# BurntSushi/suffix

Hardware: AMD Instinct MI355X
Metric: MB of input text/sec for SuffixTable::new (SA-IS+LCP), 1 GPU; bit-exact SA (higher is better)
Workload: dtype u32; 1 GPU; 100000000 B synthetic DNA (sigma=4, uniform, splitmix64) per GPU, u32 indices, device-resident text -> device SA; text_bytes_total=100000000

## Files before the change

### suffix_amd/csrc/sfx_radix.hip

```cpp
#include <stdio.h>
#include <type_traits>
#include <stdlib.h>

#include "sfx_host.hpp"

namespace sfx {

constexpr uint32_t kStatusAgg = 1u << 30;
constexpr uint32_t kStatusPrefix = 2u << 30;
constexpr uint32_t kStatusValue = (1u << 30) - 1u;
constexpr int kMaxPasses = 8;
constexpr unsigned kHistAllGrid = 1024;

struct SrcE64 {
    static constexpr bool kHasVal = false;
    static constexpr bool kFromText = false;
    const uint64_t* in;
    __device__ __forceinline__ uint64_t key(uint64_t i) const { return in[i]; }
    __device__ __forceinline__ uint32_t val(uint64_t) const { return 0u; }
};
struct SrcText32 {
    static constexpr bool kHasVal = false;
    static constexpr bool kFromText = true;
    PackedText t;
// ... 929 lines not shown
            if (owner) {
                uint32_t run = ex;
#pragma unroll
                for (int k = 0; k < NW; k++) {
                    s.cnt[k][tid] = (uint16_t)run;
                    run += c[k];
                }
                real_count = tile_count - ((tid == 255u) ? (uint32_t)(kTile - nvalid) : 0u);
                tile_ex = ex;
                if (real_count) mine = atomicAdd(&cursor[SUB ? ((top << 8) | tid) : (top * kRadix + tid) * kCursorPad], real_count);
            }
        }
        __syncthreads();
#pragma unroll
        for (int r = 0; r < KPT; r++) s.stage[pos[r] + s.cnt[w][digit_of(key[r], shift, 255u)]] = key[r];
        if (owner) s.off[tid] = mine - tile_ex;
        __syncthreads();
        constexpr int kOut = (KPT % 4 == 0) ? 4 : ((KPT % 2 == 0) ? 2 : 1);
        unsigned t = tid;
        SFX_OPAQUE_VGPR(t);
#pragma unroll
        for (int r0 = 0; r0 < KPT; r0 += kOut) {
#pragma unroll
            for (int r = r0; r < r0 + kOut; r++) key[r] = s.stage[r * kThreads + t];
#pragma unroll
            for (int r = r0; r < r0 + kOut; r++) pos[r] = s.off[digit_of(key[r], shift, 255u)] + ((unsigned)r * kThreads + t);
#pragma unroll
            for (int r = r0; r < r0 + kOut; r++)
                if ((unsigned)r * kThreads + t < nvalid) out[pos[r]] = key[r];
        }
        if (owner) {
#pragma unroll
            for (int k = 0; k < NW; k++) s.cnt[k][tid] = 0;
        }
        __syncthreads();
    }
}
constexpr int kH16Bins = 1 << 16;
constexpr int kH16Words = kH16Bins / 2;
constexpr int kH16Threads = 1024;
struct H16Zero {
    uint32_t* a;
    uint32_t na;
    uint32_t* b;
    uint32_t nb;
    __device__ __forceinline__ void clear(unsigned threads) const
    {
        for (uint32_t i = blockIdx.x * threads + threadIdx.x; i < na; i += gridDim.x * threads) a[i] = 0;
        for (uint32_t i = blockIdx.x * threads + threadIdx.x; i < nb; i += gridDim.x * threads) b[i] = 0;
    }
};
__global__ void __launch_bounds__(kH16Threads)
k_hist16_text(PackedText t, int drop, uint64_t words_per_block, uint32_t* __restrict__ partial, H16Zero z)
{
    z.clear(kH16Threads);
    __shared__ uint32_t h[kH16Words];
    const unsigned tid = threadIdx.x;
    const uint64_t nwords = (t.n + (uint64_t)t.spw - 1) / (uint64_t)t.spw;
    const uint64_t qb = (uint64_t)blockIdx.x * words_per_block;
    const uint64_t qe = dmin<uint64_t>(nwords, qb + words_per_block);
    const uint64_t mask = (1ull << t.kbits) - 1ull;
    for (unsigned i = tid; i < (unsigned)kH16Words; i += kH16Threads) h[i] = 0;
    __syncthreads();
    uint32_t w0 = 0, w1 = 0;
    if (qb + tid < qe) { w0 = t.words[qb + tid]; w1 = t.words[qb + tid + 1]; }
    for (uint64_t q = qb + tid; q < qe; q += kH16Threads) {
        const uint64_t both = ((uint64_t)w0 << t.kbits) | (uint64_t)w1;
        if (q + kH16Threads < qe) { w0 = t.words[q + kH16Threads]; w1 = t.words[q + kH16Threads + 1]; }
        const uint64_t j0 = q * (uint64_t)t.spw;
        for (int o = 0; o < t.spw; o++) {
            if (j0 + (uint64_t)o >= t.n) break;
            const uint32_t key = (uint32_t)((both >> ((unsigned)(t.spw - o) * (unsigned)t.bits)) & mask);
            const uint32_t top = key >> drop;
            atomicAdd(&h[top >> 1], (top & 1u) ? 65536u : 1u);
        }
    }
    __syncthreads();
    uint32_t* out = partial + (uint64_t)blockIdx.x * kH16Words;
    for (unsigned i = tid; i < (unsigned)kH16Words; i += kH16Threads) out[i] = h[i];
}
__global__ void __launch_bounds__(kH16Threads)
k_hist16_e64(const uint64_t* __restrict__ E, uint64_t m, int shift, uint64_t per_block, uint32_t* __restrict__ partial, H16Zero z)
{
    z.clear(kH16Threads);
    __shared__ uint32_t h[kH16Words];
    const unsigned tid = threadIdx.x;
    const uint64_t qb = (uint64_t)blockIdx.x * per_block;
    const uint64_t qe = dmin<uint64_t>(m, qb + per_block);
    for (unsigned i = tid; i < (unsigned)kH16Words; i += kH16Threads) h[i] = 0;
    __syncthreads();
    constexpr int kFly = 8;
    for (uint64_t q0 = qb; q0 < qe; q0 += (uint64_t)kH16Threads * kFly) {
        uint64_t e[kFly];
#pragma unroll
        for (int k = 0; k < kFly; k++) {
            const uint64_t q = q0 + (uint64_t)k * kH16Threads + tid;
            e[k] = q < qe ? E[q] : ~0ull;
        }
#pragma unroll
        for (int k = 0; k < kFly; k++) {
            if (q0 + (uint64_t)k * kH16Threads + tid < qe) {
                const uint32_t top = (uint32_t)(e[k] >> shift) & 0xFFFFu;
                atomicAdd(&h[top >> 1], (top & 1u) ? 65536u : 1u);
            }
        }
    }
    __syncthreads();
    uint32_t* out = partial + (uint64_t)blockIdx.x * kH16Words;
    for (unsigned i = tid; i < (unsigned)kH16Words; i += kH16Threads) out[i] = h[i];
}
struct OversizeEntry { uint32_t bin, start, size, off; };
constexpr uint32_t kOversizeMax = 16384;
constexpr int kH16FinThreads = 512;
constexpr int kH16FinBins = 4 * kH16FinThreads;
constexpr int kH16FinHalf = kH16Bins / 2;
constexpr int kH16FinPer = kH16FinHalf / kH16FinThreads;
__global__ void __launch_bounds__(kH16FinThreads)
k_hist16_finish(const uint32_t* __restrict__ partial, unsigned nblocks, unsigned rows_per_class, uint32_t* bins,
                uint32_t* class_top8, uint32_t* ticket, uint32_t* __restrict__ totals_lo, uint32_t* __restrict__ totals_hi,
                uint32_t* __restrict__ stat_out, uint32_t cap, uint32_t fast, uint32_t* __restrict__ cursor16,
                uint32_t* __restrict__ cursor8, PostTicket post)
{
    constexpr int kWaves = kH16FinThreads / kWave;
    __shared__ uint32_t tile[kH16FinHalf + kH16FinHalf / kH16FinPer];
    __shared__ uint32_t lo[kRadix];
    __shared__ uint32_t part[kWaves];
    __shared__ uint32_t sstat[5];
    __shared__ uint32_t last;
    const unsigned tid = threadIdx.x;
    {
        constexpr unsigned kGroups = kH16Bins / kH16FinBins;
        const unsigned bx = blockIdx.x % kGroups, by = blockIdx.x / kGroups;
        const unsigned w0 = bx * (kH16FinBins / 2) + tid * 2;
        uint32_t c[4] = {0, 0, 0, 0};
        const unsigned g1 = dmin(nblocks, (by + 1u) * rows_per_class);
        constexpr int kFly = 4;
        for (unsigned g = by * rows_per_class; g < g1; g += kFly) {
            uint2 v[kFly];
#pragma unroll
            for (int k = 0; k < kFly; k++) {
                v[k] = uint2{0u, 0u};
                if (g + (unsigned)k < g1) v[k] = *reinterpret_cast<const uint2*>(partial + (uint64_t)(g + (unsigned)k) * kH16Words + w0);
            }
#pragma unroll
            for (int k = 0; k < kFly; k++) {
                c[0] += v[k].x & 0xFFFFu;
                c[1] += v[k].x >> 16;
                c[2] += v[k].y & 0xFFFFu;
                c[3] += v[k].y >> 16;
            }
        }
#pragma unroll
        for (int k = 0; k < 4; k++)
            if (c[k]) atomicAdd(&bins[2 * w0 + k], c[k]);
        uint32_t all = c[0] + c[1] + c[2] + c[3];
        for (int d = 32; d >= 1; d >>= 1) all += __shfl_xor(all, d);
        static_assert(kWave * 4 == kRadix, "a wave's bins are one top-8 bucket");
        if (lane_id() == 0) class_top8[by * kRadix + (2u * w0) / (unsigned)kRadix] = all;
    }
    __builtin_amdgcn_fence(__ATOMIC_RELEASE, "agent");
    __syncthreads();
    if (tid == 0) last = (atomicAdd(ticket, 1u) == gridDim.x - 1u) ? 1u : 0u;
    __syncthreads();
    if (!last) return;
    __builtin_amdgcn_fence(__ATOMIC_ACQUIRE, "agent");
    if (tid < (unsigned)kRadix) lo[tid] = 0;
    if (tid < 5u) sstat[tid] = 0;
    uint32_t lo4[4] = {0, 0, 0, 0}, carry = 0;
    uint32_t most = 0, slow = 0, nover = 0, sover = 0;
    auto padded = [](unsigned i) { return i + i / (unsigned)kH16FinPer; };
    for (int h = 0; h < 2; h++) {
        uint32_t* const src = bins + h * kH16FinHalf;
        __syncthreads();
#pragma unroll 4
        for (int k = 0; k < kH16FinPer / 4; k++) {
            const unsigned i = (unsigned)k * kH16FinBins + 4u * tid;
            const uint4 v = *reinterpret_cast<const uint4*>(src + i);
            lo4[0] += v.x; lo4[1] += v.y; lo4[2] += v.z; lo4[3] += v.w;
            const unsigned at = padded(i);
            tile[at] = v.x; tile[at + 1] = v.y; tile[at + 2] = v.z; tile[at + 3] = v.w;
        }
        __syncthreads();
        uint32_t* const mine = tile + padded(tid * kH16FinPer);
        uint32_t sum = 0;
        for (int j = 0; j < kH16FinPer; j++) {
            const uint32_t x = mine[j];
            sum += x;
            most = dmax(most, x);
            if (x > fast) slow += x;
            if (x > cap) { nover++; sover += x; }
        }
        const uint32_t incl = wave_scan_add(sum);
        if (lane_id() == 63) part[wave_id()] = incl;
        __syncthreads();
        uint32_t run = carry + incl - sum, total = 0;
        for (unsigned k = 0; k < (unsigned)kWaves; k++) {
            if (k < wave_id()) run += part[k];
            total += part[k];
        }
        carry += total;
        static_assert(kRadix % kH16FinPer == 0, "a top-8 bucket begins with a thread's first bin");
        if ((tid * kH16FinPer) % (unsigned)kRadix == 0u) {
            const unsigned j = ((unsigned)h * kH16FinHalf + tid * kH16FinPer) / (unsigned)kRadix;
            uint32_t at = run;
            for (unsigned x = 0; x < kPartClasses; x++) {
                cursor8[(x * kRadix + j) * kCursorPad] = at;
                at += class_top8[x * kRadix + j];
            }
            totals_hi[j] = at - run;
        }
        for (int j = 0; j < kH16FinPer; j++) {
            const uint32_t x = mine[j];
            mine[j] = run;
            run += x;
        }
        __syncthreads();
#pragma unroll 4
        for (int k = 0; k < kH16FinPer / 4; k++) {
            const unsigned i = (unsigned)k * kH16FinBins + 4u * tid, at = padded(i);
            const uint4 v = uint4{tile[at], tile[at + 1], tile[at + 2], tile[at + 3]};
            *reinterpret_cast<uint4*>(src + i) = v;
            *reinterpret_cast<uint4*>(cursor16 + h * kH16FinHalf + i) = v;
        }
    }
#pragma unroll
    for (int k = 0; k < 4; k++) atomicAdd(&lo[(4u * tid + (unsigned)k) % (unsigned)kRadix], lo4[k]);
    atomicMax(&sstat[0], most);
    if (slow) atomicAdd(&sstat[4], slow);
    if (nover) { atomicAdd(&sstat[2], nover); atomicAdd(&sstat[3], sover); }
    __syncthreads();
    if (tid < (unsigned)kRadix) totals_lo[tid] = lo[tid];
    if (tid == 0) {
        bins[kH16Bins] = carry;
        const uint32_t words[5] = {sstat[0], carry, sstat[2], sstat[3], sstat[4]};
        for (int k = 0; k < 5; k++) stat_out[k] = words[k];
        post_words_from_kernel(post, words, 5u);
    }
}
__global__ void __launch_bounds__(kH16Threads)
k_hist16_oversize(const uint32_t* __restrict__ bstart, uint32_t cap, OversizeEntry* __restrict__ over)
{
    __shared__ uint64_t pover[kH16Threads / kWave];
    constexpr int kPer = kH16Bins / kH16Threads;
    const unsigned tid = threadIdx.x;
    uint64_t ov = 0;
    for (int j = 0; j < kPer; j++) {
        const uint32_t b = tid * kPer + j, v = bstart[b + 1] - bstart[b];
        if (v > cap) ov += (1ull << 32) | (uint64_t)v;
    }
    const uint64_t incl = wave_scan_add(ov);
    if (lane_id() == 63) pover[wave_id()] = incl;
    __syncthreads();
    uint64_t run = incl - ov;
    for (unsigned k = 0; k < wave_id(); k++) run += pover[k];
    if (ov == 0) return;
    for (int j = 0; j < kPer; j++) {
        const uint32_t b = tid * kPer + j, start = bstart[b], v = bstart[b + 1] - start;
        if (v > cap) {
            const uint32_t at = (uint32_t)(run >> 32);
            if (at < kOversizeMax) over[at] = OversizeEntry{b, start, v, (uint32_t)run};
            run += (1ull << 32) | (uint64_t)v;
        }
    }
}
__global__ void __launch_bounds__(kBlock)
k_oversize_gather(const uint64_t* __restrict__ X, const OversizeEntry* __restrict__ over, uint32_t nover, int low_bits,
                  uint64_t* __restrict__ T)
{
    const uint32_t lmask = (uint32_t)((1ull << low_bits) - 1ull);
    for (uint32_t j = blockIdx.x; j < nover; j += gridDim.x) {
        const OversizeEntry e = over[j];
        for (uint32_t i = threadIdx.x; i < e.size; i += kBlock) {
            const uint64_t x = X[(uint64_t)e.start + i];
            const uint32_t key = (j << low_bits) | ((uint32_t)(x >> 32) & lmask);
            T[(uint64_t)e.off + i] = ((uint64_t)key << 32) | (x & 0xFFFFFFFFull);
        }
    }
}
__global__ void __launch_bounds__(kBlock)
k_oversize_return(const uint64_t* __restrict__ T, const OversizeEntry* __restrict__ over, uint32_t nover, int low_bits,
                  uint32_t* __restrict__ K, uint32_t* __restrict__ V)
{
    const uint32_t lmask = (uint32_t)((1ull << low_bits) - 1ull);
    for (uint32_t j = blockIdx.x; j < nover; j += gridDim.x) {
        const OversizeEntry e = over[j];
        for (uint32_t i = threadIdx.x; i < e.size; i += kBlock) {
            const uint64_t x = T[(uint64_t)e.off + i];
            K[(uint64_t)e.start + i] = (e.bin << low_bits) | ((uint32_t)(x >> 32) & lmask);
            V[(uint64_t)e.start + i] = (uint32_t)x;
        }
    }
}

constexpr uint32_t kPairLimit = 32;
constexpr int kGroupBits = 10;
constexpr int kGroups = 1 << kGroupBits;
template <int WORDS, bool ON>
struct TieSmem {
    uint32_t tmask[WORDS + 1];
};
template <int WORDS>
struct TieSmem<WORDS, false> {};
template <int NW, int KPT, bool TIES = false, bool TIE_KEYS = false>
__global__ void __launch_bounds__(NW * kWave) SFX_WAVES_PER_EU(NW == 4 && KPT == 8 ? 6 : 1, 8)
k_bucket_sort(const uint64_t* __restrict__ X, const uint32_t* __restrict__ bstart, uint32_t nbuckets, int low_bits,
              uint32_t lo, uint32_t hi, uint32_t* __restrict__ K, uint32_t* __restrict__ V, uint32_t* __restrict__ GT = nullptr,
              int sbits_arg = 32)
{
    constexpr int kThreads = NW * kWave;
    constexpr uint32_t kCap = kThreads * KPT;
    constexpr int kMaskWords = (int)(kCap / 32u);
    const int sbits = TIES ? sbits_arg : 32;
    const uint64_t smask = (1ull << sbits) - 1ull;
    static_assert(kWave * KPT >= kRadix, "the match masks must fit the staging buffer");
    static_assert(NW * kRadix >= kGroups && kGroups % (NW * kWave) == 0, "the group counts of the fast path live in cnt");
    static_assert(kMaskWords < kThreads, "one thread per mask word");
    __shared__ struct {
        uint32_t cnt[NW][kRadix];
        uint16_t gstart[kGroups];
        uint32_t part[2][NW];
        uint32_t big;
        uint64_t stage[NW * kWave * KPT];
        TieSmem<kMaskWords, TIES> tie;
    } s;
    const unsigned tid = threadIdx.x, lane = lane_id(), w = wave_id();
    const unsigned long long mybit = 1ull << lane;
    const bool owner = tid < (unsigned)kRadix;
    if (tid == 0) s.big = 0u;
    unsigned long long* const my_flags = reinterpret_cast<unsigned long long*>(s.stage) + w * kRadix;
    unsigned par = 0;
    if (owner) {
#pragma unroll
        for (int k = 0; k < NW; k++) s.cnt[k][tid] = 0u;
    }
    if constexpr (TIES) {
        if (tid <= (unsigned)kMaskWords) s.tie.tmask[tid] = 0u;
    }
    __syncthreads();
    auto bounds = [&](uint32_t b, uint32_t& begin, uint32_t& size) {
        begin = 0; size = 0;
        if (b < nbuckets) { begin = bstart[b]; size = bstart[b + 1] - begin; }
        if (size <= lo || size > hi || size > kCap) size = 0;
    };
    uint64_t nkey[KPT];
    auto fetch = [&](uint32_t begin, uint32_t size) {
        const unsigned per = ((size + kThreads - 1) / kThreads) * kWave;
#pragma unroll
        for (int r = 0; r < KPT; r++) {
            const unsigned idx = w * per + r * kWave + lane;
            nkey[r] = ((unsigned)(r * kWave) < per && idx < size) ? X[(uint64_t)begin + idx] : ~0ull;
        }
    };
    uint32_t b = blockIdx.x, begin, size, begin1, size1;
    bounds(b, begin, size);
    bounds(b + gridDim.x, begin1, size1);
    fetch(begin, size);
    for (; b < nbuckets; b += gridDim.x) {
        uint64_t key[KPT];
        uint32_t pos[KPT];
#pragma unroll
        for (int r = 0; r < KPT; r++) key[r] = nkey[r];
        uint32_t begin2, size2;
        bounds(b + 2 * gridDim.x, begin2, size2);
        fetch(begin1, size1);
        const unsigned kpt = (size + kThreads - 1) / kThreads;
        const unsigned per = kpt * kWave;
        bool pairs = false;
        const uint32_t tshift = begin & 31u;
        auto tie_masks_out = [&]() {
          if constexpr (TIES) {
            const uint32_t words = (tshift + size + 31u) >> 5;
            if (tid < words) {
                const uint64_t at = (uint64_t)(begin >> 5) + tid;
                const uint32_t mt = s.tie.tmask[tid];
                if (tid == 0 || tid + 1u == words) {
                    if (mt) atomicOr(&GT[at], mt);
                } else {
                    GT[at] = mt;
                }
                s.tie.tmask[tid] = 0u;
            }
          }
        };
        if (size > 1) {
            const int gbits = low_bits < kGroupBits ? low_bits : kGroupBits;
            const int gshift = sbits + low_bits - gbits;
            const unsigned gmask = (1u << gbits) - 1u;
            uint32_t* const gcount = &s.cnt[0][0];
#pragma unroll
            for (int r = 0; r < KPT; r++)
                if ((unsigned)r < kpt && w * per + r * kWave + lane < size) pos[r] = atomicAdd(&gcount[digit_of(key[r], gshift, gmask)], 1u);
            __syncthreads();
            constexpr int kPerThread = kGroups / kThreads;
            uint32_t c[kPerThread], sum = 0, most = 0;
#pragma unroll
            for (int k = 0; k < kPerThread; k++) {
                c[k] = gcount[tid * kPerThread + k];
                sum += c[k];
                most = dmax(most, c[k]);
            }
            uint32_t run = block_scan_excl_1b<NW>(sum, s.part, par);
#pragma unroll
            for (int k = 0; k < kPerThread; k++) {
                s.gstart[tid * kPerThread + k] = (uint16_t)run;
                run += c[k];
            }
            if (most > kPairLimit) s.big = 1u;
            __syncthreads();
            pairs = s.big == 0u;
            if (pairs) {
#pragma unroll
                for (int r = 0; r < KPT; r++)
                    if ((unsigned)r < kpt && w * per + r * kWave + lane < size)
                        s.stage[s.gstart[digit_of(key[r], gshift, gmask)] + pos[r]] = key[r];
                __syncthreads();
                if constexpr (TIES) {
                    for (unsigned q = tid; q < size; q += kThreads) {
                        const uint64_t e = s.stage[q];
                        const unsigned d = digit_of(e, gshift, gmask);
                        const unsigned gb = s.gstart[d], ge = gb + gcount[d];
                        unsigned rank = 0, same = 0;
                        for (unsigned j = gb; j < ge; j++) {
                            const uint64_t x = s.stage[j];
                            rank += x < e ? 1u : 0u;
                            same += ((x ^ e) >> sbits) == 0ull ? 1u : 0u;
                        }
                        const unsigned place = gb + rank;
                        V[(uint64_t)begin + place] = (uint32_t)(e & smask);
                        if constexpr (TIE_KEYS) K[(uint64_t)begin + place] = (uint32_t)(e >> 32);
                        if (same > 1u) {
                            const unsigned bitp = tshift + place;
                            atomicOr(&s.tie.tmask[bitp >> 5], 1u << (bitp & 31u));
                        }
                    }
                } else {
                for (unsigned q = tid; q < size; q += kThreads) {
                    const uint64_t e = s.stage[q];
                    const unsigned d = digit_of(e, gshift, gmask);
                    const unsigned gb = s.gstart[d], ge = gb + gcount[d];
                    unsigned rank = 0;
                    for (unsigned j = gb; j < ge; j++) rank += s.stage[j] < e ? 1u : 0u;
                    K[(uint64_t)begin + gb + rank] = (uint32_t)(e >> 32);
                    V[(uint64_t)begin + gb + rank] = (uint32_t)e;
                }
                }
            }
            __syncthreads();
#pragma unroll
            for (int k = 0; k < kPerThread; k++) gcount[tid * kPerThread + k] = 0u;
            if (tid == 0) s.big = 0u;
            if (pairs) tie_masks_out();
            __syncthreads();
        }
        for (int pass = 0; pass < 3 && size > 1 && !pairs; pass++) {
            const int shift = sbits + 8 * pass;
            const int nb = low_bits - 8 * pass < 8 ? low_bits - 8 * pass : 8;
            if (nb <= 0) break;
            const unsigned mask = (1u << nb) - 1u;
#pragma unroll
            for (int k = 0; k < kRadix / kWave; k++) my_flags[k * kWave + lane] = 0ull;
            wave_sync();
#pragma unroll
            for (int r = 0; r < KPT; r++)
                if ((unsigned)r < kpt) pos[r] = rank_round(digit_of(key[r], shift, mask), my_flags, s.cnt[w], mybit);
            __syncthreads();
            {
                uint32_t c[NW], tile_count = 0;
#pragma unroll
                for (int k = 0; k < NW; k++) {
                    c[k] = owner ? s.cnt[k][tid] : 0u;
                    tile_count += c[k];
                }
                const uint32_t ex = block_scan_excl_1b<NW>(tile_count, s.part, par);
                if (owner) {
                    uint32_t run = ex;
#pragma unroll
                    for (int k = 0; k < NW; k++) {
                        s.cnt[k][tid] = run;
                        run += c[k];
                    }
                }
            }
            __syncthreads();
#pragma unroll
            for (int r = 0; r < KPT; r++)
                if ((unsigned)r < kpt) s.stage[pos[r] + s.cnt[w][digit_of(key[r], shift, mask)]] = key[r];
            __syncthreads();
#pragma unroll
            for (int r = 0; r < KPT; r++)
                if ((unsigned)r < kpt) key[r] = s.stage[w * per + r * kWave + lane];
            if (owner) {
#pragma unroll
                for (int k = 0; k < NW; k++) s.cnt[k][tid] = 0u;
            }
            __syncthreads();
        }
#pragma unroll
        for (int r = 0; r < KPT; r++) {
            const unsigned idx = w * per + r * kWave + lane;
            if ((unsigned)r < kpt && idx < size && !pairs) {
                V[(uint64_t)begin + idx] = (uint32_t)(key[r] & smask);
                if constexpr (TIES) {
                    if constexpr (TIE_KEYS) K[(uint64_t)begin + idx] = (uint32_t)(key[r] >> 32);
                    if (size > 1u) {
                        const uint64_t kk = key[r] >> sbits;
                        const bool eq_prev = idx > 0u && (s.stage[idx - 1u] >> sbits) == kk;
                        const bool eq_next = idx + 1u < size && (s.stage[idx + 1u] >> sbits) == kk;
                        if (eq_prev || eq_next) {
                            const unsigned bitp = tshift + idx;
                            atomicOr(&s.tie.tmask[bitp >> 5], 1u << (bitp & 31u));
                        }
                    }
                } else {
                    K[(uint64_t)begin + idx] = (uint32_t)(key[r] >> 32);
                }
            }
        }
        if constexpr (TIES) {
            if (size > 1u && !pairs) {
                __syncthreads();
                tie_masks_out();
            }
        }
        begin = begin1; size = size1;
        begin1 = begin2; size1 = size2;
    }
}

static bool radix_sweep_allowed()
{
    static const bool v = [] { const char* e = dev_env("SFX_RADIX_SWEEP"); return !e || atoi(e) != 0; }();
    return v;
}
static bool radix_kv12_allowed()
{
    static const bool v = [] { const char* e = dev_env("SFX_RADIX_KV12"); return !e || atoi(e) != 0; }();
    return v;
}

uint64_t radix_scratch_words(uint64_t m)
{
    return (uint64_t)kMaxPasses * kRadix * kHistAllGrid + (uint64_t)kMaxPasses * kRadix + 64 + m / 8 + 2 * kRadix;
}

struct RadixScratch {
    uint32_t* partial;
    uint32_t* totals;
    uint32_t* tickets;
    uint32_t* status;
    RadixScratch(uint32_t* base, uint64_t)
    {
        partial = base;
        totals = partial + (uint64_t)kMaxPasses * kRadix * kHistAllGrid;
        tickets = totals + (uint64_t)kMaxPasses * kRadix;
        status = tickets + 64;
    }
};

constexpr int kPassNW = 16;
template <class Src>
constexpr bool kDuoSrc = Src::kHasVal && !Src::kFromText && !std::is_same<Src, SrcKeyIota>::value;
template <class Src>
constexpr int kSweepKPT = !Src::kHasVal ? 16 : (Src::kFromText ? 8 : 12);
template <class Src>
constexpr int kChunkedKPT = !Src::kHasVal ? 11 : 8;

template <class Src, class Dst>
static int run_pass(const char* name, double algo_bytes, const Src& src, const Dst& dst, uint64_t m, int shift,
                    unsigned mask, const RadixScratch& scr, int pass, bool sweep, hipStream_t st)
{
    if (!sweep) {
        constexpr int kThreads = kPassNW * kWave, kTile = kThreads * kChunkedKPT<Src>;
        Chunking ch = make_chunking(m, kTile);
        const uint64_t chunk = ch.tiles_per_block * kTile;
        SFX_LAUNCH("radix_hist", (double)m * 8.0, (k_radix_hist_chunk<Src>), ch.blocks, kBlock, st, src, m, shift,
                   mask, chunk, scr.partial);
        SFX_LAUNCH("radix_scan", (double)kRadix * ch.blocks * 8, k_radix_scan, kRadix, kBlock, st, scr.partial,
                   ch.blocks, scr.totals);
        SFX_LAUNCH(name, algo_bytes, (k_radix_pass<Src, Dst, kChunkedKPT<Src>, false, kPassNW>), ch.blocks, kThreads, st, src,
                   dst, m, shift, mask, chunk, (const uint32_t*)scr.partial, (const uint32_t*)scr.totals,
                   (uint32_t*)nullptr, (uint32_t*)nullptr);
        return SFX_OK;
    }
    constexpr int kThreads = kDuoSrc<Src> ? kDuoNW * kWave : kPassNW * kWave;
    constexpr int kTile = kThreads * (kDuoSrc<Src> ? kDuoKPT : kSweepKPT<Src>);
    const uint64_t tiles = (m + kTile - 1) / kTile;
    const unsigned grid = (unsigned)dmin<uint64_t>(tiles, kMaxGrid);
    SFX_HIP(hipMemsetAsync(scr.status, 0, tiles * kRadix * sizeof(uint32_t), st));
    if constexpr (kDuoSrc<Src>) {
        SFX_LAUNCH(name, algo_bytes, (k_radix_sweep_duo<Src, Dst, kDuoKPT, kDuoNW>), grid, kThreads, st, src, dst, m, shift,
                   mask, (const uint32_t*)(scr.totals + pass * kRadix), scr.status, scr.tickets + pass);
    } else {
        SFX_LAUNCH(name, algo_bytes, (k_radix_sweep<Src, Dst, kSweepKPT<Src>, kPassNW>), grid, kThreads, st, src, dst, m, shift, mask,
                   (const uint32_t*)(scr.totals + pass * kRadix), scr.status, scr.tickets + pass);
    }
    return SFX_OK;
}

template <class Src>
static int prepare_sweep(const char* name, double algo_bytes, const Src& src, uint64_t m, int bit_lo, int bit_hi,
                         int npass, const RadixScratch& scr, hipStream_t st)
{
    Chunking ch = make_chunking(m, kBlock * 8, kHistAllGrid);
    const uint64_t chunk = ch.tiles_per_block * kBlock * 8;
    SFX_HIP(hipMemsetAsync(scr.tickets, 0, 64 * sizeof(uint32_t), st));
    SFX_LAUNCH(name, algo_bytes, (k_radix_hist_all<Src>), ch.blocks, kBlock, st, src, m, bit_lo, bit_hi, npass, chunk,
               scr.partial);
    SFX_LAUNCH("radix_scan", (double)npass * kRadix * ch.blocks * 8, k_radix_scan, npass * kRadix, kBlock, st,
               scr.partial, ch.blocks, scr.totals);
    return SFX_OK;
}

static bool window_hist_applies(const PackedText* text, uint64_t m, int bit_lo, int bit_hi)
{
    return text && m == text->n && text->kbits == 32 && (8 % text->bits) == 0 && bit_lo == 32 && bit_hi == 64;
}
static int prepare_sweep_windows(const PackedText& t, const RadixScratch& scr, hipStream_t st)
{
    const uint64_t npos = t.n + 3ull * (8 / t.bits);
    const uint64_t nwords = (npos + t.spw - 1) / t.spw;
    Chunking ch = make_chunking(nwords, kBlock * 4, kHistAllGrid);
    const uint64_t wpb = ch.tiles_per_block * kBlock * 4;
    SFX_HIP(hipMemsetAsync(scr.tickets, 0, 64 * sizeof(uint32_t), st));
    SFX_LAUNCH("radix_hist_all_text_u32", (double)t.n * t.bits / 8.0, k_window_hist, ch.blocks, kBlock, st, t, npos, wpb,
               scr.partial);
    SFX_LAUNCH("radix_scan", (double)kRadix * ch.blocks * 8, k_radix_scan, kRadix, kBlock, st, scr.partial, ch.blocks,
               scr.totals);
    SFX_LAUNCH("radix_window_fix", 0.0, k_window_fix, 1, kBlock, st, t, scr.totals);
    return SFX_OK;
}

static bool use_sweep(uint64_t m, int npass)
{
    return radix_sweep_allowed() && m < (1ull << 30) && npass <= kMaxPasses;
}

constexpr int kBucketNW = 16, kBucketKPT = 16;
static bool hybrid_size_ok(uint64_t m)
{
    static const int enabled = [] { const char* e = dev_env("SFX_HYBRID"); return e ? atoi(e) : 1; }();
    static const uint64_t min_m = [] { const char* e = dev_env("SFX_HYBRID_MIN"); return e ? (uint64_t)strtoull(e, nullptr, 10) : (1ull << 25); }();
    return enabled && m >= min_m && m <= (1ull << 28);
}
bool radix_e64_hybrid_expected(uint64_t m, int key_bits)
{
    return hybrid_size_ok(m) && key_bits >= 24;
}
static int hybrid_sort_e64_text(uint64_t* e0, uint64_t* e1, uint64_t m, int bit_lo, int bit_hi, const RadixScratch& scr,
                                hipStream_t st, sfx_build_stats* stats, const PackedText& text, uint32_t* split_v,
                                uint32_t** split_k_out, bool* done, bool* windows_ready, int elem_bits = 0, TieRecords* ties = nullptr)
{
    if (ties) ties->produced = false;
    *done = false;
    *windows_ready = false;
    const bool from_elems = elem_bits > 0;
    static const uint32_t cap = [] {
        const char* e = dev_env("SFX_HYBRID_CAP");
        const uint32_t full = kBucketNW * kWave * kBucketKPT;
        const uint32_t v = e ? (uint32_t)atoi(e) : full;
        return v >= 1 && v < full ? v : full;
    }();
    const int key_bits = from_elems ? elem_bits : bit_hi - bit_lo;
    if (!hybrid_size_ok(m) || bit_lo != 32 || key_bits < 24 || key_bits > bit_hi - bit_lo) return SFX_OK;
    if (!from_elems && (key_bits != text.kbits || m != text.n)) return SFX_OK;
    const int low_bits = key_bits - 16;
    const int top_hi = bit_lo + key_bits;
    constexpr uint64_t kReserve = 1u << 18;
    uint32_t* bins = scr.partial + ((uint64_t)kMaxPasses * kRadix * kHistAllGrid - kReserve);
    uint32_t* stat = bins + kH16Bins + 64;
    OversizeEntry* over = reinterpret_cast<OversizeEntry*>(bins + kH16Bins + 128);
    static_assert(kH16Bins + 128 + 4 * kOversizeMax <= kReserve, "the reserve holds bins, statistics and the oversize list");
    uint32_t* partial = reinterpret_cast<uint32_t*>(e1);
    const uint64_t nwords = from_elems ? m : (m + (uint64_t)text.spw - 1) / (uint64_t)text.spw;
    const uint64_t room = m * sizeof(uint64_t) / (kH16Words * sizeof(uint32_t));
    if (room == 0) return SFX_OK;
    Chunking ch = make_chunking(nwords, kH16Threads, (unsigned)dmin<uint64_t>(room, 256));
    const H16Zero zero = {bins, (uint32_t)(kH16Bins + 128), scr.tickets, 64u};
    if (from_elems)
        SFX_LAUNCH("radix_hist16_elems", (double)m * 8.0, k_hist16_e64, ch.blocks, kH16Threads, st, (const uint64_t*)e0, m, top_hi - 16,
                   ch.tiles_per_block * kH16Threads, partial, zero);
    else
        SFX_LAUNCH("radix_hist16_text", (double)m * text.bits / 8.0, k_hist16_text, ch.blocks, kH16Threads, st, text, low_bits,
                   ch.tiles_per_block * kH16Threads, partial, zero);
    const unsigned rows_per_class = (ch.blocks + kPartClasses - 1) / kPartClasses;
    const uint64_t class_len = (uint64_t)rows_per_class * ch.tiles_per_block * kH16Threads * (from_elems ? 1u : (uint64_t)text.spw);
    uint32_t* cursor16 = bins + kH16Bins + 128 + 4 * kOversizeMax;
    uint32_t* class_top8 = cursor16 + kH16Bins;
    uint32_t* cursor8 = class_top8 + kPartClasses * kRadix;
    static_assert(kH16Bins + 128 + 4 * kOversizeMax + kH16Bins + kPartClasses * kRadix * (1 + kCursorPad) <= kReserve, "the reserve holds the cursors too");
    uint32_t host_stat[5] = {0, 0, 0, 0, 0};
    const PostTicket post = post_ticket();
    SFX_LAUNCH("radix_hist16_finish", (double)ch.blocks * kH16Words * 4 + (double)kH16Bins * 12, k_hist16_finish,
               (kH16Bins / kH16FinBins) * kPartClasses, kH16FinThreads, st, (const uint32_t*)partial, ch.blocks, rows_per_class, bins, class_top8,
               stat + 16, scr.totals, scr.totals + kRadix, stat, cap, dmin(cap, 4096u), cursor16, cursor8, post);
    SFX_TRY(read_posted(host_stat, stat, sizeof(host_stat), post, st));
    const uint32_t host_max = host_stat[0], nover = host_stat[2];
    const uint64_t nlarge = host_stat[3], nslow = host_stat[4];
    const bool give_way = nover > kOversizeMax || nslow * 64 > m ||
                          (nover && (m + 1) / 2 + 32 + 2 * (nlarge + 32) > m);
    if ((uint64_t)host_stat[1] != m) return SFX_OK;
    if (give_way) {
        if (!from_elems && text.kbits == 32 && (8 % text.bits) == 0 && bit_hi == 64) {
            SFX_HIP(hipMemsetAsync(scr.tickets, 0, 64 * sizeof(uint32_t), st));
            SFX_LAUNCH("radix_window_from_hist16", 0.0, k_window_from_hist16, 1, kBlock, st, scr.totals, (uint32_t)(3 * (8 / text.bits)));
            SFX_LAUNCH("radix_window_fix", 0.0, k_window_fix, 1, kBlock, st, text, scr.totals);
            *windows_ready = true;
        }
        return SFX_OK;
    }
    static const int ties_on = [] { const char* e = dev_env("SFX_HYBRID_TIES"); return e ? atoi(e) : 1; }();
    const bool tie_mode = ties && ties_on && nover == 0;
    static const int partition = [] { const char* e = dev_env("SFX_HYBRID_PARTITION"); return e ? atoi(e) : 1; }();
    static const int key36_on = [] { const char* e = dev_env("SFX_HYBRID_KEY36"); return e ? atoi(e) : 1; }();
    int extra = 0;
    if (tie_mode && key36_on && partition && !from_elems && text.kbits == 32 && text.bits <= 4 && m <= (1ull << 28))
        extra = key36_on >= 2 ? (4 / text.bits) * text.bits : text.bits;
    const bool wide_key = extra > text.bits;
    const int sbits = 32 - extra;
    if (partition) {
        constexpr int kPKpt = 16;
        static const unsigned cus = [] {
            int dev = 0, n = 0;
            if (hipGetDevice(&dev) != hipSuccess || hipDeviceGetAttribute(&n, hipDeviceAttributeMultiprocessorCount, dev) != hipSuccess || n <= 0) n = 256;
            return (unsigned)n;
        }();
        static const int pwaves = [] { const char* e = dev_env("SFX_PARTITION_WAVES"); const int v = e ? atoi(e) : 8; return (v == 16 || v == 4) ? v : 8; }();
        auto partition_pair = [&](auto nw) -> int {
            constexpr int kPNw = decltype(nw)::value;
            const uint64_t tile = (uint64_t)kPKpt * kPNw * kWave;
            const unsigned per_cu = 16u / kPNw;
            const unsigned g1 = (unsigned)dmin<uint64_t>((m + tile - 1) / tile, dmin(per_cu * cus, grid_cap()));
            const unsigned g2 = (unsigned)dmin<uint64_t>((m + tile - 1) / tile + kRadix, dmin(per_cu * cus, grid_cap()));
            if (from_elems) {
                SFX_LAUNCH("radix_scatter_u32", (double)m * 16.0, (k_partition<SrcE64, kPKpt, kPNw, false>), g1, kPNw * kWave, st,
                           SrcE64{e0}, e1, m, top_hi - 8, cursor8, (const uint32_t*)bins, class_len);
                SFX_LAUNCH("radix_scatter_u32", (double)m * 16.0, (k_partition<SrcE64, kPKpt, kPNw, true>), g2, kPNw * kWave, st,
                           SrcE64{e1}, e0, m, top_hi - 16, cursor16, (const uint32_t*)bins, class_len);
                uint64_t* t = e0; e0 = e1; e1 = t;
            } else {
                const int loader_spw = (kPNw == 8 && text.bits * text.spw == 32 && text.kbits == 32 && !wide_key &&
                                        class_len % (uint64_t)text.spw == 0) ? text.spw : 0;
                auto text_pass = [&](auto tsrc, auto spw) -> int {
                    SFX_LAUNCH("radix_scatter_text_u32", (double)m * (text.bits / 8.0 + 8.0),
                               (k_partition<decltype(tsrc), kPKpt, kPNw, false, (kPNw == 8 ? decltype(spw)::value : 0)>), g1, kPNw * kWave, st,
                               tsrc, e0, m, top_hi - 8, cursor8, (const uint32_t*)bins, class_len);
                    return SFX_OK;
                };
                auto text_pass_of = [&](auto tsrc) -> int {
                    switch (loader_spw) {
                    case 32: return text_pass(tsrc, std::integral_constant<int, 32>{});
                    case 16: return text_pass(tsrc, std::integral_constant<int, 16>{});
                    case 8: return text_pass(tsrc, std::integral_constant<int, 8>{});
                    case 4: return text_pass(tsrc, std::integral_constant<int, 4>{});
                    default: return text_pass(tsrc, std::integral_constant<int, 0>{});
                    }
                };
                if (extra) SFX_TRY(text_pass_of(SrcText36{text, extra, wide_key}));
                else SFX_TRY(text_pass_of(SrcText32{text}));
                SFX_LAUNCH("radix_scatter_u32", (double)m * 16.0, (k_partition<SrcE64, kPKpt, kPNw, true>), g2, kPNw * kWave, st,
                           SrcE64{e0}, e1, m, top_hi - 16, cursor16, (const uint32_t*)bins, class_len);
            }
            return SFX_OK;
        };
        if (pwaves == 16) SFX_TRY(partition_pair(std::integral_constant<int, 16>{}));
        else if (pwaves == 4) SFX_TRY(partition_pair(std::integral_constant<int, 4>{}));
        else SFX_TRY(partition_pair(std::integral_constant<int, 8>{}));
    } else if (from_elems) {
        SFX_TRY(run_pass("radix_scatter_u32", (double)m * 16.0, SrcE64{e0}, DstE64{e1}, m, top_hi - 16, 255u, scr, 0, true, st));
        SFX_TRY(run_pass("radix_scatter_u32", (double)m * 16.0, SrcE64{e1}, DstE64{e0}, m, top_hi - 8, 255u, scr, 1, true, st));
        uint64_t* t = e0; e0 = e1; e1 = t;
    } else {
        SrcText32 tsrc = {text};
        SFX_TRY(run_pass("radix_scatter_text_u32", (double)m * (text.bits / 8.0 + 8.0), tsrc, DstE64{e0}, m, top_hi - 16, 255u, scr, 0,
                         true, st));
        SFX_TRY(run_pass("radix_scatter_u32", (double)m * 16.0, SrcE64{e0}, DstE64{e1}, m, top_hi - 8, 255u, scr, 1, true, st));
    }
    uint32_t* split_k = reinterpret_cast<uint32_t*>(e0);
    const uint64_t* over_sorted = nullptr;
    if (nover) {
        SFX_LAUNCH("radix_hist16_oversize", (double)kH16Bins * 8, k_hist16_oversize, 1, kH16Threads, st, (const uint32_t*)bins, cap, over);
        uint64_t* T = e0 + (((m + 1) / 2 + 31) & ~uint64_t(31));
        uint64_t* T2 = T + ((nlarge + 31) & ~uint64_t(31));
        const unsigned g = (unsigned)dmin<uint64_t>(nover, kMaxGrid);
        SFX_LAUNCH("oversize_gather", (double)nlarge * 16, k_oversize_gather, g, kBlock, st, (const uint64_t*)e1, (const OversizeEntry*)over,
                   nover, low_bits, T);
        int in1 = 0;
        SFX_TRY(radix_sort_e64(T, T2, nlarge, 32, 32 + low_bits + bits_for(nover > 1 ? nover - 1 : 1), scr.partial, st, &in1, stats,
                               nullptr, nullptr, nullptr, 0));
        over_sorted = in1 ? T2 : T;
    }
    static const int force_geom = [] { const char* e = dev_env("SFX_HYBRID_GEOM"); return e ? atoi(e) : -1; }();
    const uint32_t top = dmin(host_max, cap);
    const uint32_t c1 = force_geom >= 1 ? 0u : dmin(2048u, cap), c2 = force_geom == 2 ? c1 : dmin(4096u, cap);
    const unsigned grid = (unsigned)dmin<uint64_t>(kH16Bins, (uint64_t)grid_cap() * 2);
    const uint64_t mask_words = ((m + 31) / 32 + 64) & ~uint64_t(31);
    const bool tie_keys = tie_mode && ties->want_keys;
    uint32_t* const gt = reinterpret_cast<uint32_t*>(e0) + (tie_keys ? ((m + 63) & ~uint64_t(63)) : 0);
    if (tie_keys && (((m + 63) & ~uint64_t(63)) + 3 * mask_words) * sizeof(uint32_t) > m * sizeof(uint64_t)) return SFX_ERR_INTERNAL;
    uint32_t* const gl = gt + mask_words;
    uint32_t* const gh = gl + mask_words;
    if (tie_mode) SFX_HIP(hipMemsetAsync(gt, 0, 2 * mask_words * sizeof(uint32_t), st));
#define SFX_BUCKET_SORT(NW, KPT, LO, HI, GRID)                                                                              \
    do {                                                                                                                    \
        if (tie_mode && tie_keys)                                                                                           \
            SFX_LAUNCH("bucket_sort_ties_keys", (double)m * 16.125, (k_bucket_sort<NW, KPT, true, true>), GRID, NW * kWave, st, (const uint64_t*)e1, \
                       (const uint32_t*)bins, (uint32_t)kH16Bins, low_bits + extra, (uint32_t)(LO), (uint32_t)(HI), split_k, split_v, gt, sbits); \
        else if (tie_mode)                                                                                                  \
            SFX_LAUNCH("bucket_sort_ties", (double)m * 12.125, (k_bucket_sort<NW, KPT, true>), GRID, NW * kWave, st, (const uint64_t*)e1, \
                       (const uint32_t*)bins, (uint32_t)kH16Bins, low_bits + extra, (uint32_t)(LO), (uint32_t)(HI), (uint32_t*)nullptr, split_v, \
                       gt, sbits);                                                                                          \
        else                                                                                                                \
            SFX_LAUNCH("bucket_sort_lds", (double)m * 16.0, (k_bucket_sort<NW, KPT>), GRID, NW * kWave, st, (const uint64_t*)e1, \
                       (const uint32_t*)bins, (uint32_t)kH16Bins, low_bits, (uint32_t)(LO), (uint32_t)(HI), split_k, split_v); \
    } while (0)
    if (c1 > 0) SFX_BUCKET_SORT(4, 8, 0u, c1, grid);
    if (c2 > c1 && top > c1) SFX_BUCKET_SORT(4, 16, c1, c2, grid);
    if (cap > c2 && top > c2) SFX_BUCKET_SORT(16, 16, c2, cap, dmin(grid, grid_cap()));
#undef SFX_BUCKET_SORT
    if (tie_mode) {
        ties->produced = true;
        ties->tmask = gt;
        ties->lmask = gl;
        ties->hmask = gh;
    }
// ... 648 lines not shown
```

Measured before the change: 78720 MB/s.

## Restructure bucket-sort fast path with packed 16-bit group counts and batched placement

```diff
diff --git a/suffix_amd/csrc/sfx_radix.hip b/suffix_amd/csrc/sfx_radix.hip
--- a/suffix_amd/csrc/sfx_radix.hip
+++ b/suffix_amd/csrc/sfx_radix.hip
@@ -1255,7 +1255,7 @@
 template <int WORDS>
 struct TieSmem<WORDS, false> {};
 template <int NW, int KPT, bool TIES = false, bool TIE_KEYS = false>
-__global__ void __launch_bounds__(NW * kWave) SFX_WAVES_PER_EU(NW == 4 && KPT == 8 ? 6 : 1, 8)
+__global__ void __launch_bounds__(NW * kWave) SFX_WAVES_PER_EU(NW == 4 ? (KPT == 8 ? 6 : 4) : 1, 8)
 k_bucket_sort(const uint64_t* __restrict__ X, const uint32_t* __restrict__ bstart, uint32_t nbuckets, int low_bits,
               uint32_t lo, uint32_t hi, uint32_t* __restrict__ K, uint32_t* __restrict__ V, uint32_t* __restrict__ GT = nullptr,
               int sbits_arg = 32)
@@ -1266,23 +1266,23 @@
     const int sbits = TIES ? sbits_arg : 32;
     const uint64_t smask = (1ull << sbits) - 1ull;
     static_assert(kWave * KPT >= kRadix, "the match masks must fit the staging buffer");
-    static_assert(NW * kRadix >= kGroups && kGroups % (NW * kWave) == 0, "the group counts of the fast path live in cnt");
+    static_assert(NW * kRadix >= kGroups && kGroups % (NW * kWave) == 0 && kCap <= 0xFFFFu, "two sets of 16-bit group counts of the fast path live in cnt");
     static_assert(kMaskWords < kThreads, "one thread per mask word");
+    constexpr int kPlaceRounds = 2, kPlaceAhead = 4;
+    constexpr uint32_t kDump = kWave;
+    static_assert(KPT % kPlaceRounds == 0 && kPlaceAhead <= (int)kDump && kPairLimit <= kDump, "the reads ahead end inside the spare words");
     __shared__ struct {
         uint32_t cnt[NW][kRadix];
         uint16_t gstart[kGroups];
         uint32_t part[2][NW];
         uint32_t big;
-        uint64_t stage[NW * kWave * KPT];
+        uint64_t stage[kCap + kDump];
         TieSmem<kMaskWords, TIES> tie;
     } s;
     const unsigned tid = threadIdx.x, lane = lane_id(), w = wave_id();
-    const unsigned long long mybit = 1ull << lane;
-    const bool owner = tid < (unsigned)kRadix;
     if (tid == 0) s.big = 0u;
-    unsigned long long* const my_flags = reinterpret_cast<unsigned long long*>(s.stage) + w * kRadix;
-    unsigned par = 0;
-    if (owner) {
+    unsigned par = 0, flip = 0;
+    if (tid < (unsigned)kRadix) {
 #pragma unroll
         for (int k = 0; k < NW; k++) s.cnt[k][tid] = 0u;
     }
@@ -1296,18 +1296,18 @@
         if (size <= lo || size > hi || size > kCap) size = 0;
     };
     uint64_t nkey[KPT];
-    auto fetch = [&](uint32_t begin, uint32_t size) {
+    auto fetch = [&](uint64_t (&to)[KPT], uint32_t begin, uint32_t size) {
         const unsigned per = ((size + kThreads - 1) / kThreads) * kWave;
 #pragma unroll
         for (int r = 0; r < KPT; r++) {
             const unsigned idx = w * per + r * kWave + lane;
-            nkey[r] = ((unsigned)(r * kWave) < per && idx < size) ? X[(uint64_t)begin + idx] : ~0ull;
+            to[r] = ((unsigned)(r * kWave) < per && idx < size) ? X[(uint64_t)begin + idx] : ~0ull;
         }
     };
     uint32_t b = blockIdx.x, begin, size, begin1, size1;
     bounds(b, begin, size);
     bounds(b + gridDim.x, begin1, size1);
-    fetch(begin, size);
+    fetch(nkey, begin, size);
     for (; b < nbuckets; b += gridDim.x) {
         uint64_t key[KPT];
         uint32_t pos[KPT];
@@ -1315,7 +1315,7 @@
         for (int r = 0; r < KPT; r++) key[r] = nkey[r];
         uint32_t begin2, size2;
         bounds(b + 2 * gridDim.x, begin2, size2);
-        fetch(begin1, size1);
+        fetch(nkey, begin1, size1);
         const unsigned kpt = (size + kThreads - 1) / kThreads;
         const unsigned per = kpt * kWave;
         bool pairs = false;
@@ -1339,10 +1339,14 @@
             const int gbits = low_bits < kGroupBits ? low_bits : kGroupBits;
             const int gshift = sbits + low_bits - gbits;
             const unsigned gmask = (1u << gbits) - 1u;
-            uint32_t* const gcount = &s.cnt[0][0];
-#pragma unroll
-            for (int r = 0; r < KPT; r++)
-                if ((unsigned)r < kpt && w * per + r * kWave + lane < size) pos[r] = atomicAdd(&gcount[digit_of(key[r], gshift, gmask)], 1u);
+            uint32_t* const gwords = &s.cnt[0][0] + flip * (kGroups / 2);
+            uint16_t* const gcount = reinterpret_cast<uint16_t*>(gwords);
+#pragma unroll
+            for (int r = 0; r < KPT; r++) {
+                const unsigned d = digit_of(key[r], gshift, gmask), half = (d & 1u) * 16u;
+                pos[r] = ((unsigned)r < kpt && w * per + r * kWave + lane < size) ? (atomicAdd(&gwords[d >> 1], 1u << half) >> half) & 0xFFFFu : 0u;
+            }
+            flip ^= 1u;
             __syncthreads();
             constexpr int kPerThread = kGroups / kThreads;
             uint32_t c[kPerThread], sum = 0, most = 0;
@@ -1362,40 +1366,74 @@
             __syncthreads();
             pairs = s.big == 0u;
             if (pairs) {
-#pragma unroll
-                for (int r = 0; r < KPT; r++)
-                    if ((unsigned)r < kpt && w * per + r * kWave + lane < size)
-                        s.stage[s.gstart[digit_of(key[r], gshift, gmask)] + pos[r]] = key[r];
+                uint32_t at[KPT];
+#pragma unroll
+                for (int r = 0; r < KPT; r++) at[r] = s.gstart[digit_of(key[r], gshift, gmask)];
+#pragma unroll
+                for (int r = 0; r < KPT; r++) {
+                    const bool live = (unsigned)r < kpt && w * per + r * kWave + lane < size;
+                    s.stage[live ? at[r] + pos[r] : kCap + lane] = key[r];
+                }
                 __syncthreads();
-                if constexpr (TIES) {
-                    for (unsigned q = tid; q < size; q += kThreads) {
-                        const uint64_t e = s.stage[q];
-                        const unsigned d = digit_of(e, gshift, gmask);
-                        const unsigned gb = s.gstart[d], ge = gb + gcount[d];
-                        unsigned rank = 0, same = 0;
-                        for (unsigned j = gb; j < ge; j++) {
-                            const uint64_t x = s.stage[j];
-                            rank += x < e ? 1u : 0u;
-                            same += ((x ^ e) >> sbits) == 0ull ? 1u : 0u;
-                        }
-                        const unsigned place = gb + rank;
-                        V[(uint64_t)begin + place] = (uint32_t)(e & smask);
-                        if constexpr (TIE_KEYS) K[(uint64_t)begin + place] = (uint32_t)(e >> 32);
-                        if (same > 1u) {
-                            const unsigned bitp = tshift + place;
-                            atomicOr(&s.tie.tmask[bitp >> 5], 1u << (bitp & 31u));
+                uint32_t* const Vb = V + begin;
+                uint32_t* const Kb = (!TIES || TIE_KEYS) ? K + begin : nullptr;
+#pragma unroll
+                for (int r0 = 0; r0 < KPT; r0 += kPlaceRounds) {
+                    if ((unsigned)r0 * kThreads >= size) break;
+                    uint64_t e[kPlaceRounds];
+                    unsigned gb[kPlaceRounds], gc[kPlaceRounds], rank[kPlaceRounds], same[kPlaceRounds], most = 0;
+#pragma unroll
+                    for (int j = 0; j < kPlaceRounds; j++) e[j] = s.stage[tid + (unsigned)(r0 + j) * kThreads];
+#pragma unroll
+                    for (int j = 0; j < kPlaceRounds; j++) {
+                        const unsigned d = digit_of(e[j], gshift, gmask);
+                        gb[j] = s.gstart[d];
+                        gc[j] = gcount[d];
+                    }
+                    uint64_t x[kPlaceRounds][kPlaceAhead];
+#pragma unroll
+                    for (int j = 0; j < kPlaceRounds; j++) {
+#pragma unroll
+                        for (int k = 0; k < kPlaceAhead; k++) x[j][k] = s.stage[gb[j] + (unsigned)k];
+                    }
+#pragma unroll
+                    for (int j = 0; j < kPlaceRounds; j++) {
+                        if (tid + (unsigned)(r0 + j) * kThreads >= size) gc[j] = 0u;
+                        most = dmax(most, gc[j]);
+                        rank[j] = 0u;
+                        same[j] = 0u;
+#pragma unroll
+                        for (int k = 0; k < kPlaceAhead; k++) {
+                            const bool in = (unsigned)k < gc[j];
+                            rank[j] += (unsigned)in & (unsigned)(x[j][k] < e[j]);
+                            if constexpr (TIES) same[j] += (unsigned)in & (unsigned)((x[j][k] ^ e[j]) <= smask);
                         }
                     }
-                } else {
-                for (unsigned q = tid; q < size; q += kThreads) {
-                    const uint64_t e = s.stage[q];
-                    const unsigned d = digit_of(e, gshift, gmask);
-                    const unsigned gb = s.gstart[d], ge = gb + gcount[d];
-                    unsigned rank = 0;
-                    for (unsigned j = gb; j < ge; j++) rank += s.stage[j] < e ? 1u : 0u;
-                    K[(uint64_t)begin + gb + rank] = (uint32_t)(e >> 32);
-                    V[(uint64_t)begin + gb + rank] = (uint32_t)e;
-                }
+#pragma unroll 1
+                    for (unsigned k = kPlaceAhead; k < most; k++) {
+                        uint64_t y[kPlaceRounds];
+#pragma unroll
+                        for (int j = 0; j < kPlaceRounds; j++) y[j] = s.stage[gb[j] + k];
+#pragma unroll
+                        for (int j = 0; j < kPlaceRounds; j++) {
+                            const bool in = k < gc[j];
+                            rank[j] += (unsigned)in & (unsigned)(y[j] < e[j]);
+                            if constexpr (TIES) same[j] += (unsigned)in & (unsigned)((y[j] ^ e[j]) <= smask);
+                        }
+                    }
+#pragma unroll
+                    for (int j = 0; j < kPlaceRounds; j++) {
+                        if (gc[j] == 0u) continue;
+                        const unsigned place = gb[j] + rank[j];
+                        Vb[place] = (uint32_t)(e[j] & smask);
+                        if constexpr (!TIES || TIE_KEYS) Kb[place] = (uint32_t)(e[j] >> 32);
+                        if constexpr (TIES) {
+                            if (same[j] > 1u) {
+                                const unsigned bitp = tshift + place;
+                                atomicOr(&s.tie.tmask[bitp >> 5], 1u << (bitp & 31u));
+                            }
+                        }
+                    }
                 }
             }
             __syncthreads();
@@ -1403,76 +1441,85 @@
             for (int k = 0; k < kPerThread; k++) gcount[tid * kPerThread + k] = 0u;
             if (tid == 0) s.big = 0u;
             if (pairs) tie_masks_out();
-            __syncthreads();
-        }
-        for (int pass = 0; pass < 3 && size > 1 && !pairs; pass++) {
-            const int shift = sbits + 8 * pass;
-            const int nb = low_bits - 8 * pass < 8 ? low_bits - 8 * pass : 8;
-            if (nb <= 0) break;
-            const unsigned mask = (1u << nb) - 1u;
-#pragma unroll
-            for (int k = 0; k < kRadix / kWave; k++) my_flags[k * kWave + lane] = 0ull;
-            wave_sync();
-#pragma unroll
-            for (int r = 0; r < KPT; r++)
-                if ((unsigned)r < kpt) pos[r] = rank_round(digit_of(key[r], shift, mask), my_flags, s.cnt[w], mybit);
-            __syncthreads();
-            {
-                uint32_t c[NW], tile_count = 0;
-#pragma unroll
-                for (int k = 0; k < NW; k++) {
-                    c[k] = owner ? s.cnt[k][tid] : 0u;
-                    tile_count += c[k];
-                }
-                const uint32_t ex = block_scan_excl_1b<NW>(tile_count, s.part, par);
-                if (owner) {
-                    uint32_t run = ex;
+            if (!pairs) __syncthreads();
+        }
+        if (!pairs) {
+            unsigned tid_again = tid;
+            SFX_OPAQUE_VGPR(tid_again);
+            const unsigned tid = tid_again, lane = tid & 63u, w = tid >> 6;
+            const unsigned long long mybit = 1ull << lane;
+            const bool owner = tid < (unsigned)kRadix;
+            unsigned long long* const my_flags = reinterpret_cast<unsigned long long*>(s.stage) + w * kRadix;
+            fetch(key, begin, size);
+            for (int pass = 0; pass < 3 && size > 1 && !pairs; pass++) {
+                const int shift = sbits + 8 * pass;
+                const int nb = low_bits - 8 * pass < 8 ? low_bits - 8 * pass : 8;
+                if (nb <= 0) break;
+                const unsigned mask = (1u << nb) - 1u;
+#pragma unroll
+                for (int k = 0; k < kRadix / kWave; k++) my_flags[k * kWave + lane] = 0ull;
+                wave_sync();
+#pragma unroll
+                for (int r = 0; r < KPT; r++)
+                    if ((unsigned)r < kpt) pos[r] = rank_round(digit_of(key[r], shift, mask), my_flags, s.cnt[w], mybit);
+                __syncthreads();
+                {
+                    uint32_t c[NW], tile_count = 0;
 #pragma unroll
                     for (int k = 0; k < NW; k++) {
-                        s.cnt[k][tid] = run;
-                        run += c[k];
+                        c[k] = owner ? s.cnt[k][tid] : 0u;
+                        tile_count += c[k];
+                    }
+                    const uint32_t ex = block_scan_excl_1b<NW>(tile_count, s.part, par);
+                    if (owner) {
+                        uint32_t run = ex;
+#pragma unroll
+                        for (int k = 0; k < NW; k++) {
+                            s.cnt[k][tid] = run;
+                            run += c[k];
+                        }
                     }
                 }
-            }
-            __syncthreads();
-#pragma unroll
-            for (int r = 0; r < KPT; r++)
-                if ((unsigned)r < kpt) s.stage[pos[r] + s.cnt[w][digit_of(key[r], shift, mask)]] = key[r];
-            __syncthreads();
-#pragma unroll
-            for (int r = 0; r < KPT; r++)
-                if ((unsigned)r < kpt) key[r] = s.stage[w * per + r * kWave + lane];
-            if (owner) {
-#pragma unroll
-                for (int k = 0; k < NW; k++) s.cnt[k][tid] = 0u;
-            }
-            __syncthreads();
-        }
-#pragma unroll
-        for (int r = 0; r < KPT; r++) {
-            const unsigned idx = w * per + r * kWave + lane;
-            if ((unsigned)r < kpt && idx < size && !pairs) {
-                V[(uint64_t)begin + idx] = (uint32_t)(key[r] & smask);
-                if constexpr (TIES) {
-                    if constexpr (TIE_KEYS) K[(uint64_t)begin + idx] = (uint32_t)(key[r] >> 32);
-                    if (size > 1u) {
-                        const uint64_t kk = key[r] >> sbits;
-                        const bool eq_prev = idx > 0u && (s.stage[idx - 1u] >> sbits) == kk;
-                        const bool eq_next = idx + 1u < size && (s.stage[idx + 1u] >> sbits) == kk;
-                        if (eq_prev || eq_next) {
-                            const unsigned bitp = tshift + idx;
-                            atomicOr(&s.tie.tmask[bitp >> 5], 1u << (bitp & 31u));
+                __syncthreads();
+#pragma unroll
+                for (int r = 0; r < KPT; r++)
+                    if ((unsigned)r < kpt) s.stage[pos[r] + s.cnt[w][digit_of(key[r], shift, mask)]] = key[r];
+                __syncthreads();
+#pragma unroll
+                for (int r = 0; r < KPT; r++)
+                    if ((unsigned)r < kpt) key[r] = s.stage[w * per + r * kWave + lane];
+                if (owner) {
+#pragma unroll
+                    for (int k = 0; k < NW; k++) s.cnt[k][tid] = 0u;
+                }
+                __syncthreads();
+            }
+#pragma unroll
+            for (int r = 0; r < KPT; r++) {
+                const unsigned idx = w * per + r * kWave + lane;
+                if ((unsigned)r < kpt && idx < size && !pairs) {
+                    V[(uint64_t)begin + idx] = (uint32_t)(key[r] & smask);
+                    if constexpr (TIES) {
+                        if constexpr (TIE_KEYS) K[(uint64_t)begin + idx] = (uint32_t)(key[r] >> 32);
+                        if (size > 1u) {
+                            const uint64_t kk = key[r] >> sbits;
+                            const bool eq_prev = idx > 0u && (s.stage[idx - 1u] >> sbits) == kk;
+                            const bool eq_next = idx + 1u < size && (s.stage[idx + 1u] >> sbits) == kk;
+                            if (eq_prev || eq_next) {
+                                const unsigned bitp = tshift + idx;
+                                atomicOr(&s.tie.tmask[bitp >> 5], 1u << (bitp & 31u));
+                            }
                         }
+                    } else {
+                        K[(uint64_t)begin + idx] = (uint32_t)(key[r] >> 32);
                     }
-                } else {
-                    K[(uint64_t)begin + idx] = (uint32_t)(key[r] >> 32);
                 }
             }
-        }
-        if constexpr (TIES) {
-            if (size > 1u && !pairs) {
-                __syncthreads();
-                tie_masks_out();
+            if constexpr (TIES) {
+                if (size > 1u && !pairs) {
+                    __syncthreads();
+                    tie_masks_out();
+                }
             }
         }
         begin = begin1; size = size1;
```

After: 79230 MB/s (median of 6 runs). About the same (+0.6%).
